# edwinyosorahardjo/compressjs-flattened

Hardware: AMD Instinct MI355X
Metric: bzip2 -9 compress MB/s at 1/2/4/8 MI355X; bit-exact output size vs ref (higher is better)
Workload: dtype u32; 1 GPU; Bzip2.compressFile level 9 (899981-byte blocks) on 1 x 100000000 bytes enwik8-shaped synthetic text (tools/textgen.c seed 1), device-resident; per_gpu_bytes=100000000, level=9, parallelism=1 GPU

## Files before the change

compressjs-flattened_amd/csrc/bwt.hip:

```cpp
#include "radix.hpp"
#include <stdlib.h>
#include <string.h>
#include <type_traits>

namespace cjs {

struct Geom { uint32_t nb, stride, n_last; };
__device__ __forceinline__ uint32_t blk_len(const Geom& g, uint32_t blk) { return blk == g.nb - 1 ? g.n_last : g.stride; }
struct VarGeom { uint32_t nb, stride, n_last; const uint32_t* len; };
__device__ __forceinline__ uint32_t blk_len(const VarGeom& g, uint32_t blk) { return g.len[blk]; }

template <typename G>
__global__ __launch_bounds__(256) void bwt_init_keys(const uint8_t* __restrict__ T, G g, int cyclic, int nsym, uint32_t M,
                                                     uint64_t* __restrict__ key, uint32_t* __restrict__ val) {
  for (uint64_t a = (uint64_t)blockIdx.x * 256 + threadIdx.x; a < M; a += (uint64_t)gridDim.x * 256) {
    const uint32_t blk = (uint32_t)(a / g.stride), i = (uint32_t)(a - (uint64_t)blk * g.stride), n = blk_len(g, blk);
    const uint8_t* t = T + (size_t)blk * g.stride;
    uint64_t k = 0;
    if constexpr (std::is_same_v<G, VarGeom>) {
      uint32_t x = i;
      if (i >= n) k = (1ull << (8 * nsym)) | i;
      else for (int j = 0; j < nsym; j++) { k = (k << 8) | t[x]; if (++x == n) x = 0; }
      k |= (uint64_t)blk << (8 * nsym + 1);
    } else if (cyclic) {
// ... 131 lines not shown
  const uint32_t single = nh & nx;
  uint32_t surv = (uint32_t)__popc(valid & ~single), heads = (uint32_t)__popc(nh & ~single);
  uint32_t last = nh ? (uint32_t)base + (uint32_t)tid * 16u + 32u - (uint32_t)__clz(nh) : 0u;
  {
    const uint64_t any = __ballot(nh != 0);
    const uint32_t run0 = (uint32_t)wave_id() * 2u;
    if (lane_id() == 0) {
      bool bad = false;
      for (uint32_t b = 0; b < 2; b++) bad |= base + (uint64_t)(run0 + b + 1u) * 512u <= A && (uint32_t)(any >> (32 * b)) == 0u;
      if (bad) atomicOr(big_flag, 1u);
    }
  }
  surv = block_sum<256>(surv, sm);
  heads = block_sum<256>(heads, sm);
  last = wave_max(last);
  if (lane_id() == 0) sm[wave_id()] = last;
  __syncthreads();
  if (tid == 0) {
    uint32_t m = sm[0]; for (int i = 1; i < 4; i++) m = sm[i] > m ? sm[i] : m;
    tile_cnt[blockIdx.x] = surv; tile_cnt[T + blockIdx.x] = heads; tile_cnt[2 * (size_t)T + blockIdx.x] = m;
  }
}

__global__ __launch_bounds__(1024) void bwt_scan_tiles(uint32_t* __restrict__ tile_cnt, uint32_t T, uint32_t* __restrict__ counters,
                                                      uint32_t* __restrict__ host_mirror ) {
  __shared__ uint32_t sm[16];
  __shared__ uint32_t mx[1024];
  uint32_t c0 = 0, c1 = 0, cm = 0;
  for (uint32_t base = 0; base < T; base += 1024) {
    const uint32_t i = base + threadIdx.x;
    const bool ok = i < T;
    uint32_t t0, t1;
    const uint32_t v0 = ok ? tile_cnt[i] : 0u, v1 = ok ? tile_cnt[T + i] : 0u, v2 = ok ? tile_cnt[2 * (size_t)T + i] : 0u;
    const uint32_t e0 = block_excl_sum<1024>(v0, sm, t0);
    const uint32_t e1 = block_excl_sum<1024>(v1, sm, t1);
    const uint32_t im = block_incl_max<1024>(v2, sm);
    mx[threadIdx.x] = im;
    __syncthreads();
    const uint32_t prev = threadIdx.x ? mx[threadIdx.x - 1] : 0u;
    const uint32_t chunk_max = mx[1023];
    __syncthreads();
    if (ok) {
      tile_cnt[i] = c0 + e0; tile_cnt[T + i] = c1 + e1;
      tile_cnt[2 * (size_t)T + i] = prev > cm ? prev : cm;
    }
    c0 += t0; c1 += t1; cm = chunk_max > cm ? chunk_max : cm;
  }
  if (threadIdx.x == 0) { counters[0] = c0; counters[1] = c1; host_mirror[0] = c0; host_mirror[1] = c1; host_mirror[4] = counters[4]; counters[4] = 0; }
}

__device__ __forceinline__ uint64_t class_head_before(const uint64_t* __restrict__ key, uint64_t seg0, uint64_t base, int shift, int lane) {
  if (base == seg0) return base;
  const uint64_t target = key[base] >> shift;
  const uint64_t off = base - seg0;
  const uint32_t back = off < 64u ? (uint32_t)off : 64u;
  const bool eq = (uint32_t)lane < back && (key[base - 1u - (uint32_t)lane] >> shift) == target;
  const uint64_t ne = ~__ballot(eq);
  const uint32_t m = ne ? (uint32_t)__builtin_ctzll(ne) : 64u;
  if (m < 64u || off <= 64u) return base - m;
  uint64_t lo = seg0, hi = base - 64u;
  while (hi > lo) {
    const uint64_t len = hi - lo, step = (len + 63u) / 64u, idx = lo + (uint64_t)lane * step;
    const bool hit = idx >= hi || (key[idx] >> shift) == target;
    const uint64_t hits = __ballot(hit);
    const uint32_t j = hits ? (uint32_t)__builtin_ctzll(hits) : 64u;
    if (!j) { hi = lo; break; }
    const uint64_t nhi = lo + (uint64_t)j * step;
    lo += (uint64_t)(j - 1u) * step + 1u;
    if (j < 64u && nhi < hi) hi = nhi;
  }
  return hi;
// ... 492 lines not shown
#pragma unroll
    for (int s = 0; s < 16; s++) {
      const uint32_t d = (comp[s] >> shift) & 255u;
      se[wcnt[w][d] + rk[s]] = ((uint64_t)comp[s] << 32) | pv[s];
    }
    __syncthreads();
#pragma unroll
    for (int s = 0; s < 16; s++) {
      const uint64_t e = se[(uint32_t)w * 1024u + (uint32_t)s * 64u + lane];
      comp[s] = (uint32_t)(e >> 32); pv[s] = (uint32_t)e;
    }
    __syncthreads();
  }
#pragma unroll
  for (int s = 0; s < 16; s++) {
    if ((ownm >> s) & 1u) {
      const uint32_t x = (uint32_t)w * 1024u + (uint32_t)s * 64u + lane;
      const uint32_t pc = x ? (uint32_t)(se[x - 1] >> 32) : ~comp[s];
      hflag[wb + x] = (uint8_t)((comp[s] != pc ? HF_NEW : 0u) | ((comp[s] >> 20) != (pc >> 20) ? HF_OLD : 0u));
      val[wb + x] = pv[s];
    }
  }
}
__global__ __launch_bounds__(1024) void scan_u32_single(uint32_t* __restrict__ arr, uint32_t n, uint32_t* __restrict__ total, uint32_t* __restrict__ host_total) {
  __shared__ uint32_t sm[16];
  uint32_t carry = 0;
  for (uint32_t base = 0; base < n; base += 1024) {
    const uint32_t i = base + threadIdx.x;
    uint32_t v = i < n ? arr[i] : 0u, tot;
    const uint32_t ex = block_excl_sum<1024>(v, sm, tot);
    if (i < n) arr[i] = carry + ex;
    carry += tot;
  }
  if (threadIdx.x == 0) { *total = carry; *host_total = carry; }
}
__device__ __forceinline__ void defer_flags(uint32_t A, const uint8_t* __restrict__ dflag, const uint64_t* __restrict__ key, uint64_t a0,
                                            uint32_t& f, uint32_t& heads, uint64_t (&k8)[8]) {
  f = 0; heads = 0;
  if (a0 >= A) return;
  if (a0 + 8 <= A) {
    const uint64_t w = *(const uint64_t*)(dflag + a0);
#pragma unroll
    for (int j = 0; j < 8; j++) f |= (uint32_t)((w >> (8 * j)) & 1ull) << j;
  } else for (int j = 0; j < 8; j++) if (a0 + j < A && dflag[a0 + j]) f |= 1u << j;
  if (!f) return;
#pragma unroll
  for (int j = 0; j < 8; j++) k8[j] = a0 + j < A ? key[a0 + j] : 0ull;
  const bool pf = a0 && dflag[a0 - 1];
  uint64_t prev = pf ? key[a0 - 1] >> 20 : ~0ull;
  bool prev_def = pf;
#pragma unroll
  for (int j = 0; j < 8; j++) {
    const bool d = (f >> j) & 1u;
    if (d && (!prev_def || prev != (k8[j] >> 20))) heads |= 1u << j;
    prev_def = d; prev = k8[j] >> 20;
  }
}
// ... 149 lines not shown
  if (tile >= Tn) return;
#pragma unroll 4
  for (int it = 0; it < 16; it++) {
    const uint64_t a = (uint64_t)tile * RS_TILE + (uint32_t)it * 256 + threadIdx.x;
    if (a >= M) break;
    const uint32_t blk = (uint32_t)(a / g.stride), p = (uint32_t)(a - (uint64_t)blk * g.stride), n = blk_len(g, blk);
    const uint8_t* t = T + (size_t)blk * g.stride;
    uint8_t* u = U + (size_t)blk * g.stride;
    const uint32_t s = __builtin_nontemporal_load(SA + a);
    const uint32_t p0 = R[(size_t)blk * g.stride];
    if (p == p0) u[0] = t[n - 1];
    else u[p < p0 ? p + 1 : p] = t[s - 1];
  }
}

enum Counter { CN_SURVIVORS = 0, CN_GROUPS = 1, CN_DEFERRED = 2, CN_DEFERRED_GROUPS = 3, CN_LARGE_GROUP = 4 };

size_t BwtWork::bytes_needed(size_t cap) {
  const size_t T = RadixWork::hist_tiles_for(cap);
  size_t b = 0;
  auto add = [&](size_t n) { b += (n + 255) & ~(size_t)255; };
  add(cap * 8); add(cap * 8); add(cap * 4); add(cap * 4); add(cap * 4); add(cap * 4); add(cap * 4);
  add(cap * 4); add(cap * 4); add(cap); add(cap);
  add(RadixWork::hist_words(T) * 4); add(256 * RadixWork::segs_for(cap) * 4); add(3 * T * 4); add(64);
  return b + 4096;
}
int BwtWork::carve(Arena& a, size_t cap_) {
  cap = cap_;
  const size_t T = RadixWork::hist_tiles_for(cap);
  key[0] = a.take<uint64_t>(cap); key[1] = a.take<uint64_t>(cap);
  val[0] = a.take<uint32_t>(cap); val[1] = a.take<uint32_t>(cap);
  pos[0] = a.take<uint32_t>(cap); pos[1] = a.take<uint32_t>(cap);
  gord = a.take<uint32_t>(cap);
  R = a.take<uint32_t>(cap); SA = a.take<uint32_t>(cap); dflag = a.take<uint8_t>(cap); hflag = a.take<uint8_t>(cap);
  CJS_TRY(rs.carve(a, T, RadixWork::segs_for(cap)));
  tile_cnt = a.take<uint32_t>(3 * T); counters = a.take<uint32_t>(16);
  if (!counters) return CJS_E_OUT_OF_MEMORY;
  if (!h_counters) CJS_HIP_TRY(hipHostMalloc((void**)h_counters.put(), 64));
  if (!ev_scan) CJS_HIP_TRY(hipEventCreateWithFlags(ev_scan.put(), hipEventDisableTiming));
  return 0;
}

struct Plan {
  bool segmented, packed;
  bool sweeps;
  int nsym, bits;
  int gs1, carried;
  SegGeom sg; GenSrc gen;
  const uint8_t* Tx; uint8_t* U;
};
template <typename G>
static Plan plan_round1(const BwtWork& w, const G& g, bool cyclic, const uint8_t* d_T, uint8_t* d_U) {
  constexpr bool VAR = std::is_same_v<G, VarGeom>;
  Plan p;
  const int sym_bits = cyclic ? 8 : 9;
  const uint32_t tps = ((g.nb > 1 ? g.stride : g.n_last) + RS_TILE - 1) / RS_TILE;
  p.segmented = !VAR && (uint64_t)g.nb * tps <= w.rs.hist_tiles && g.nb <= w.rs.bintot_segs && getenv("CJS_NO_SEGMENTED_SORT") == nullptr;
  p.packed = p.segmented && cyclic;
  p.sweeps = g.nb >= 8 && p.packed;
// ... 28 lines not shown
  hipLaunchKernelGGL(bwt_phase2_records, dim3(p.sg.nseg * p.sg.tps), dim3(256), 0, s, w.key[r.c], p.sg, p.gen.T, w.rs.hist, w.key[1 - r.c]);
  r.c = 1 - r.c;
  return radix_passes<uint64_t>(s, w.rs, w.key[0], w.val[0], w.key[1], w.val[1], r.c, r.A, 48, 64, lt, &p.sg, nullptr, true, true, w.dflag);
}

template <typename TG>
static void launch_tile_sort(hipStream_t s, uint32_t Tt, uint64_t* key, uint32_t* val, uint8_t* hflag, uint32_t A, uint8_t* dflag, uint32_t ngroups, const TG& tg) {
  if (ngroups && A / ngroups >= 5) hipLaunchKernelGGL(bwt_tile_sort_radix<TG>, dim3(xcd_grid(Tt)), dim3(256), 0, s, key, val, hflag, A, dflag, tg, Tt);
  else hipLaunchKernelGGL(bwt_tile_sort<TG>, dim3(xcd_grid(Tt)), dim3(256), 0, s, key, val, hflag, A, dflag, tg, Tt);
}
static int sort_round_whole(hipStream_t s, BwtWork& w, Round& r, LaunchTimes* lt) {
  CJS_TRY((radix_passes<uint64_t>(s, w.rs, w.key[0], w.val[0], w.key[1], w.val[1], r.c, r.A, 0, r.bits, lt)));
  hipLaunchKernelGGL(bwt_key_flags, dim3((r.A + 255) / 256 < 8192u ? (r.A + 255) / 256 : 8192u), dim3(256), 0, s, w.key[r.c], r.A, w.hflag);
  CJS_HIP_TRY(hipGetLastError());
  return 0;
}
static bool tile_sorted_round(uint32_t A) { return A >= 2 * TS_WIN; }
template <typename TG>
static int sort_round(hipStream_t s, BwtWork& w, Round& r, LaunchTimes* lt, const TG& tg) {
  if (!tile_sorted_round(r.A)) return sort_round_whole(s, w, r, lt);
  const uint32_t A = r.A, Tt = (A + TS_NOM - 1) / TS_NOM, Tg = (A + TS_GT - 1) / TS_GT;
  const int c = r.c;
  uint8_t* dflag = w.dflag;
  uint32_t* tcount = w.tile_cnt;
  if (r.no_large_groups) {
    launch_tile_sort(s, Tt, w.key[c], w.val[c], w.hflag, A, nullptr, r.ngroups, tg);
    CJS_HIP_TRY(hipGetLastError());
    return 0;
  }
  dev_fill(s, dflag, 1, A);
  launch_tile_sort(s, Tt, w.key[c], w.val[c], w.hflag, A, dflag, r.ngroups, tg);
  uint32_t* hcount = w.rs.hist;
  hipLaunchKernelGGL(bwt_defer_count, dim3(Tg), dim3(256), 0, s, A, dflag, w.key[c], tcount, hcount);
  hipLaunchKernelGGL(scan_u32_single, dim3(1), dim3(1024), 0, s, hcount, Tg, w.counters + CN_DEFERRED_GROUPS, w.h_counters + CN_DEFERRED_GROUPS);
  hipLaunchKernelGGL(scan_u32_single, dim3(1), dim3(1024), 0, s, tcount, Tg, w.counters + CN_DEFERRED, w.h_counters + CN_DEFERRED);
  CJS_HIP_TRY(hipStreamSynchronize(s));
  const uint32_t D = w.h_counters[CN_DEFERRED];
  if (env_debug()) fprintf(stderr, "[cjs bwt]   tile sort: %u of %u suffixes in groups > %u\n", D, A, TS_MAXGRP);
  if (D == 0) { r.no_large_groups = true; return 0; }
  if ((size_t)D > w.cap / 2) {
    const uint32_t Tk = (A + RS_TILE - 1) / RS_TILE;
    hipLaunchKernelGGL(bwt_gather_keys<decltype(tg.g)>, dim3(xcd_grid(Tk)), dim3(256), 0, s, tg.g, tg.cyclic, A, tg.h, tg.R, w.val[c], tg.pos, tg.gord, w.key[c], Tk);
    return sort_round_whole(s, w, r, lt);
  }
  uint64_t* dk0 = w.key[1 - c]; uint64_t* dk1 = dk0 + w.cap / 2;
  uint32_t* dv0 = w.val[1 - c]; uint32_t* dv1 = dv0 + w.cap / 2;
  uint32_t* dpos = w.pos[1 - r.pc];
  hipLaunchKernelGGL(bwt_defer_gather, dim3(Tg), dim3(256), 0, s, w.key[c], w.val[c], A, dflag, tcount, hcount, dk0, dv0, dpos);
  int cur = 0;
  const uint32_t ndg = w.h_counters[CN_DEFERRED_GROUPS];
  CJS_TRY((radix_passes<uint64_t>(s, w.rs, dk0, dv0, dk1, dv1, cur, D, 0, 20 + bits_for(ndg ? ndg - 1 : 0), lt)));
  hipLaunchKernelGGL(bwt_defer_scatter, dim3((D + 255) / 256 < 8192u ? (D + 255) / 256 : 8192u), dim3(256), 0, s, D, cur ? dk1 : dk0, cur ? dv1 : dv0, dpos,
                     w.hflag, w.val[c]);
  CJS_HIP_TRY(hipGetLastError());
  return 0;
}

template <bool FIRST, bool PACKED, int SWEEP, typename G>
static void launch_apply(hipStream_t s, BwtWork& w, const G& g, const Plan& p, const Round& r, uint32_t T) {
  hipLaunchKernelGGL((bwt_apply<FIRST, PACKED, SWEEP, G>), dim3(xcd_grid(T)), dim3(256), 0, s, FIRST ? w.key[r.c] : nullptr, FIRST ? nullptr : w.hflag,
                     w.val[r.c], w.pos[r.pc], r.A, g, w.tile_cnt, T, w.R, w.SA, w.val[1 - r.c], w.pos[1 - r.pc], w.gord, HalfMap{SWEEP ? 2u : 1u, g.stride},
                     p.Tx, p.U, w.counters + CN_LARGE_GROUP, p.gs1, p.carried);
}
template <typename G>
static int regroup(hipStream_t s, BwtWork& w, const G& g, const Plan& p, const Round& r) {
  const uint32_t T = (r.A + RS_TILE - 1) / RS_TILE;
  const bool first = r.rounds == 0, sweeps = first && p.sweeps;
  if (sweeps) launch_apply<true, true, 1>(s, w, g, p, r, T);
  else if (first) hipLaunchKernelGGL(bwt_flags, dim3(T), dim3(256), 0, s, w.key[r.c], r.A, w.tile_cnt, T, p.gs1, w.counters + CN_LARGE_GROUP, g.stride);
  else hipLaunchKernelGGL(bwt_flags_bytes, dim3(T), dim3(256), 0, s, w.hflag, r.A, w.tile_cnt, T, w.counters + CN_LARGE_GROUP);
  hipLaunchKernelGGL(bwt_scan_tiles, dim3(1), dim3(1024), 0, s, w.tile_cnt, T, w.counters, w.h_counters);
  CJS_HIP_TRY(hipEventRecord(w.ev_scan, s));
  if (sweeps) launch_apply<true, true, 2>(s, w, g, p, r, T);
  else if (first && p.packed) launch_apply<true, true, 0>(s, w, g, p, r, T);
  else if (first) launch_apply<true, false, 0>(s, w, g, p, r, T);
  else launch_apply<false, false, 0>(s, w, g, p, r, T);
  return 0;
}

template <typename G>
static void prepare_next(hipStream_t s, BwtWork& w, const G& g, bool cyclic, Round& r, TsGatherT<G>& tg) {
  if (tile_sorted_round(r.A)) tg = TsGatherT<G>{w.R, w.pos[r.pc], w.gord, r.h, (int)cyclic, g};
  else {
    const uint32_t Tg = (r.A + RS_TILE - 1) / RS_TILE;
    hipLaunchKernelGGL(bwt_gather_keys<G>, dim3(xcd_grid(Tg)), dim3(256), 0, s, g, (int)cyclic, r.A, r.h, w.R, w.val[r.c], w.pos[r.pc], w.gord, w.key[r.c], Tg);
  }
  r.h = r.h < (1u << 29) ? r.h * 2 : r.h;
  r.bits = 20 + bits_for(r.ngroups ? r.ngroups - 1 : 0);
}

template <typename G>
static int bwt_run_impl(hipStream_t s, BwtWork& w, const uint8_t* d_T, const G g, bool cyclic, uint8_t* d_U, uint32_t* d_pidx,
                        cjs_stats* stats, bool resolve_stats) {
  constexpr bool VAR = std::is_same_v<G, VarGeom>;
// ... 61 lines not shown
```

compressjs-flattened_amd/csrc/cjs_internal.h:

```cpp
#pragma once
#include <hip/hip_runtime.h>
#include <stdint.h>
#include <stddef.h>
#include <stdio.h>
#include <new>
#include "cjs_hip.h"

#define CJS_HIP_TRY(expr)                                                                   \
  do {                                                                                      \
    hipError_t _e = (expr);                                                                 \
    if (_e != hipSuccess) {                                                                 \
      fprintf(stderr, "[cjs_hip] %s failed: %s (%s:%d)\n", #expr, hipGetErrorString(_e), __FILE__, __LINE__); \
      return _e == hipErrorOutOfMemory ? CJS_E_OUT_OF_MEMORY : CJS_E_HIP;                    \
    }                                                                                       \
  } while (0)
#define CJS_TRY(expr) do { int _rc = (expr); if (_rc) return _rc; } while (0)

namespace cjs {

void clear_detail();
void set_detail(const char* fmt, ...);
bool env_debug(); bool env_no_ctx_cache();

#define CJS_GUARD_BEGIN try {
// ... 127 lines not shown
  }
};

struct SegGeom; struct GenSrc;
template <typename K>
int radix_passes(hipStream_t s, RadixWork& w, K* k0, uint32_t* v0, K* k1, uint32_t* v1, int& cur, uint32_t n, int lo_bit, int hi_bit,
                 LaunchTimes* lt = nullptr, const SegGeom* seg = nullptr, const GenSrc* gen = nullptr, bool noval = false,
                 bool first_hist_ready = false, uint8_t* dig = nullptr);
int radix_pass_segments(hipStream_t s, RadixWork& w, uint32_t* k0, uint32_t* v0, uint32_t* k1, uint32_t* v1, int& cur, uint32_t nseg, uint32_t stride,
                        int lo_bit, int hi_bit, bool noval, bool first_hist_ready);

struct BwtWork {
  size_t cap = 0;
  uint64_t* key[2] = {nullptr, nullptr};
  uint32_t* val[2] = {nullptr, nullptr};
  uint32_t* pos[2] = {nullptr, nullptr};
  uint32_t* gord = nullptr;
  uint32_t* R = nullptr;
  uint32_t* SA = nullptr;
  uint8_t* dflag = nullptr;
  uint8_t* hflag = nullptr;
  RadixWork rs;
  uint32_t* tile_cnt = nullptr;
  uint32_t* counters = nullptr;
  Pinned<uint32_t> h_counters;
  Event ev_scan;
  LaunchTimes lt;
  static size_t bytes_needed(size_t cap);
  int carve(Arena& a, size_t cap);
};

int bwt_run(hipStream_t s, BwtWork& w, const uint8_t* d_T, uint32_t nb, uint32_t stride, uint32_t n_last,
            bool cyclic, uint8_t* d_U, uint32_t* d_pidx, cjs_stats* stats, bool resolve_stats = true);
int bwt_run_var(hipStream_t s, BwtWork& w, const uint8_t* d_T, uint32_t nb, uint32_t stride, const uint32_t* d_len,
                uint8_t* d_U, uint32_t* d_pidx);
int ibwt_sentinel_run(hipStream_t s, const uint8_t* d_T, uint32_t max_len, uint32_t nb, const uint32_t* lens, const uint32_t* pidx, uint8_t* d_out);
struct MtfBufs;
int bwtc_model_launch(hipStream_t s, bool fast, const MtfBufs& mb, uint32_t nb, uint64_t* d_steps, size_t step_stride, uint32_t* d_nsteps);

}
```

compressjs-flattened_amd/csrc/huff.hip:

```cpp
#include "cjs_internal.h"
#include "prims.hpp"
#include "huff.h"

namespace cjs {

constexpr int MAXSYM = 258;
constexpr int MAX_BITS = 20;
constexpr int GSZ = 50;
constexpr int PD_GROUPS = 80;

__device__ uint64_t g_huff_clk[32];
__device__ uint64_t g_bt_clk[8];
#define BT_MARK(i) do { if (blockIdx.x == 0 && threadIdx.x == 0) g_bt_clk[i] = wall_clock64(); } while (0)
#define HB_MARK(i) do { if (dbg && blockIdx.x == 0 && threadIdx.x == 0) g_huff_clk[i] = wall_clock64(); } while (0)

__device__ __forceinline__ int ha_mod(int x, int len) { return x >= len ? x - len : x; }
__device__ __forceinline__ int ha_first(const int* a, int len, int i, int nodes_to_move) {
  const int limit = i;
  int k = len - 2;
  while (i >= nodes_to_move && ha_mod(a[i], len) > limit) { k = i; i -= (limit - i + 1); }
  if (i < nodes_to_move - 1) i = nodes_to_move - 1;
  while (k > i + 1) {
    const int mid = (i + k) >> 1;
    if (ha_mod(a[mid], len) > limit) k = mid; else i = mid;
// ... 252 lines not shown
          atomicAdd(&rep[(e1 / GSZ == gc ? sc : sd) * 260 + (ys[q] >> 16)], 1u);
        }
      }
    }
    if (i_hi >= npos) for (uint32_t i = nv * 8 + threadIdx.x; i < npos; i += 1024) atomicAdd(&rep[sel[i / GSZ] * 260 + A[i]], 1u);
  }
}

__device__ void block_accounting(HuffShared& S, HuffBufs& hb, uint32_t blk, const uint8_t* __restrict__ sel, uint8_t* __restrict__ selj,
                                 const uint16_t* __restrict__ bcost, const uint8_t* __restrict__ alist_all, uint32_t nsel, uint32_t asz, int n, int ng) {
  uint32_t data_bits = 0;
  {
    const uint32_t ntile = (nsel + PD_GROUPS - 1) / PD_GROUPS;
    uint32_t tsum = 0;
    if (threadIdx.x < ntile) {
      const uint32_t g1 = (threadIdx.x + 1) * PD_GROUPS < nsel ? (threadIdx.x + 1) * PD_GROUPS : nsel;
      for (uint32_t g = threadIdx.x * PD_GROUPS; g < g1; g++) tsum += bcost[g];
    }
    const uint32_t tex = block_excl_sum<1024>(tsum, S.sm, data_bits);
    if (threadIdx.x < ntile) hb.tileoff[(size_t)blk * hb.tile_stride + threadIdx.x] = tex;
  }
  uint32_t sel_bits = 0;
  {
    uint32_t lastc[6] = {0, 0, 0, 0, 0, 0};
    for (uint32_t base = 0; base < nsel; base += 1024) {
      const uint32_t g = base + threadIdx.x;
      const uint32_t sv = g < nsel ? sel[g] : 255u;
      uint32_t lastv[6];
#pragma unroll
      for (int v = 0; v < 6; v++) {
        const uint32_t mine = sv == (uint32_t)v ? g + 1 : 0u;
        const uint32_t im = block_incl_max<1024>(mine, S.sm);
        S.chist[threadIdx.x] = im;
        __syncthreads();
        const uint32_t ex = threadIdx.x ? S.chist[threadIdx.x - 1] : 0u;
        const uint32_t tmax = S.chist[1023];
        __syncthreads();
        lastv[v] = ex > lastc[v] ? ex : lastc[v];
        lastc[v] = tmax > lastc[v] ? tmax : lastc[v];
      }
      if (g < nsel) {
        uint32_t j = 0, mylast = 0;
#pragma unroll
        for (int v = 0; v < 6; v++) if ((uint32_t)v == sv) mylast = lastv[v];
#pragma unroll
        for (int v = 0; v < 6; v++) {
          if (v >= ng || (uint32_t)v == sv) continue;
          if (mylast) j += lastv[v] > mylast;
          else j += (lastv[v] != 0) || ((uint32_t)v < sv);
        }
        selj[g] = (uint8_t)j;
        sel_bits += j + 1;
      }
    }
  }
  sel_bits = block_sum<1024>(sel_bits, S.sm);
  uint32_t tab_bits = 0;
  for (int i = threadIdx.x; i < ng * n; i += 1024) {
    const int t = i / n, s = i - t * n;
    const int cur = S.lens[t][s], prev = s ? S.lens[t][s - 1] : cur;
    tab_bits += 2u * (uint32_t)(cur > prev ? cur - prev : prev - cur) + 1u + (s == 0 ? 5u : 0u);
  }
  tab_bits = block_sum<1024>(tab_bits, S.sm);
  if (threadIdx.x < 8) S.counts[threadIdx.x] = 0;
  __syncthreads();
  if (threadIdx.x < asz) atomicOr(&S.counts[0], 1u << (alist_all[(size_t)blk * 256 + threadIdx.x] >> 4));
  __syncthreads();
  const uint32_t nranges = (uint32_t)__builtin_popcount(S.counts[0]);
  uint8_t* glens = hb.lens + (size_t)blk * 6 * MAXSYM;
  uint32_t* gcodes = hb.codes + (size_t)blk * 6 * MAXSYM;
  for (int i = threadIdx.x; i < 6 * 32; i += 1024) (&S.key[0][0])[i] = 0;
  __syncthreads();
  uint32_t* lhist = &S.key[0][0];
  for (int i = threadIdx.x; i < ng * n; i += 1024) { const int t = i / n, s = i - t * n; atomicAdd(&lhist[t * 32 + S.lens[t][s]], 1u); }
  __syncthreads();
  if (threadIdx.x < (uint32_t)ng) {
// ... 445 lines not shown
```

compressjs-flattened_amd/csrc/prims.hpp:

```cpp
#pragma once
#include <hip/hip_runtime.h>
#include <stdint.h>

namespace cjs {

constexpr int WAVE = 64;

__device__ __forceinline__ int lane_id() { return threadIdx.x & 63; }
__device__ __forceinline__ int wave_id() { return threadIdx.x >> 6; }

template <int CTRL, int ROW_MASK>
__device__ __forceinline__ uint32_t dpp_move(uint32_t idv, uint32_t x) {
  return (uint32_t)__builtin_amdgcn_update_dpp((int)idv, (int)x, CTRL, ROW_MASK, 0xF, false);
}
constexpr int DPP_ROW_SHR1 = 0x111, DPP_ROW_SHR2 = 0x112, DPP_ROW_SHR4 = 0x114, DPP_ROW_SHR8 = 0x118, DPP_ROW_BCAST15 = 0x142, DPP_ROW_BCAST31 = 0x143;

template <typename Op>
__device__ __forceinline__ uint32_t wave_incl_scan_dpp(uint32_t x, uint32_t idv, Op op) {
  x = op(x, dpp_move<DPP_ROW_SHR1, 0xF>(idv, x));
  x = op(x, dpp_move<DPP_ROW_SHR2, 0xF>(idv, x));
  x = op(x, dpp_move<DPP_ROW_SHR4, 0xF>(idv, x));
  x = op(x, dpp_move<DPP_ROW_SHR8, 0xF>(idv, x));
  x = op(x, dpp_move<DPP_ROW_BCAST15, 0xA>(idv, x));
  x = op(x, dpp_move<DPP_ROW_BCAST31, 0xC>(idv, x));
// ... 81 lines not shown
    T s = lane < NW ? smem[lane] : T(0);
    s = wave_incl_max(s);
    if (lane < NW) smem[lane] = s;
  }
  __syncthreads();
  if (w) { T b = smem[w - 1]; incl = b > incl ? b : incl; }
  __syncthreads();
  return incl;
}
template <int BLOCK, typename T>
__device__ __forceinline__ T block_sum(T v, T* smem) {
  constexpr int NW = BLOCK / 64;
  const int lane = lane_id(), w = wave_id();
  T s = wave_sum(v);
  if (lane == 0) smem[w] = s;
  __syncthreads();
  T r = T(0);
#pragma unroll
  for (int i = 0; i < NW; i++) r += smem[i];
  __syncthreads();
  return r;
}

static __global__ __launch_bounds__(256) void dev_fill_kernel(uint4* __restrict__ p, uint32_t word, size_t n16) {
  const uint4 v = make_uint4(word, word, word, word);
  for (size_t i = (size_t)blockIdx.x * 256 + threadIdx.x; i < n16; i += (size_t)gridDim.x * 256) p[i] = v;
}
static inline void dev_fill(hipStream_t s, void* p, uint8_t byte, size_t bytes) {
  const size_t n16 = (bytes + 15) / 16;
  if (!n16) return;
  const size_t wg = (n16 + 255) / 256;
  hipLaunchKernelGGL(dev_fill_kernel, dim3((unsigned)(wg < 4096 ? wg : 4096)), dim3(256), 0, s, (uint4*)p, 0x01010101u * byte, n16);
}

}
```

compressjs-flattened_amd/csrc/radix.hip:

```cpp
#include "radix.hpp"

namespace cjs {

constexpr int HR = 8;
template <typename K, bool GEN>
__global__ __launch_bounds__(256) void rs_hist(const K* __restrict__ keys, SegGeom sg, GenSrc gs, int shift,
                                               uint32_t* __restrict__ hist, uint32_t T) {
  __shared__ uint32_t h[4 * 256 * HR];
  __shared__ __attribute__((aligned(16))) uint8_t tb[GEN ? RS_TILE + GEN_PAD + 16 : 16];
  const int tid = threadIdx.x;
  uint32_t* hw = h + (tid >> 6) * 256 * HR + (tid & (HR - 1));
#pragma unroll
  for (int i = 0; i < 4 * HR; i++) h[i * 256 + tid] = 0;
  const uint32_t tile = blockIdx.x;
  const TileRef t = tile_ref(sg, tile);
  uint32_t tb0 = 0;
  if (GEN) tb0 = gen_stage(gs, sg, t, tb);
  __syncthreads();
  if (GEN) {
#pragma unroll 4
    for (int it = 0; it < 16; it++) {
      const uint32_t loc = (uint32_t)it * 256 + tid;
      if (loc < t.nvalid) atomicAdd(&hw[((uint32_t)(gen_key(gs, sg, t, tb, tb0, loc) >> shift) & 255u) * HR], 1u);
    }
// ... 38 lines not shown
  uint32_t wv[5];
#pragma unroll
  for (int j = 0; j < 5; j++) {
    const uint32_t wi = (uint32_t)j * 256u + tid;
    wv[j] = (t.nvalid && (uintptr_t)(al + wi) < a1) ? al[wi] : 0u;
  }
  __syncthreads();
#pragma unroll
  for (int j = 0; j < 5; j++) {
    const uintptr_t wa = (uintptr_t)(al + ((uint32_t)j * 256u + tid));
#pragma unroll
    for (int b = 0; b < 4; b++)
      if (wa + b >= a0 && wa + b < a1) atomicAdd(&hw[((wv[j] >> (8 * b)) & 255u) * HB], 1u);
  }
  __syncthreads();
  uint32_t sum = 0;
#pragma unroll
  for (int i = 0; i < 4; i++)
#pragma unroll
    for (int r = 0; r < HB; r++) sum += h[i * 256 * HB + tid * HB + r];
  hist[(size_t)tile * 256 + tid] = sum;
}

__global__ __launch_bounds__(256) void rs_scan_bins(uint32_t* __restrict__ hist, uint32_t tps, uint32_t* __restrict__ bintot) {
  uint32_t* p = hist + (size_t)blockIdx.x * tps * 256 + threadIdx.x;
  uint32_t carry = 0;
  uint32_t i = 0;
  for (; i + 8 <= tps; i += 8) {
    uint32_t v[8];
#pragma unroll
    for (int j = 0; j < 8; j++) v[j] = p[(size_t)(i + j) * 256];
#pragma unroll
    for (int j = 0; j < 8; j++) { p[(size_t)(i + j) * 256] = carry; carry += v[j]; }
  }
  for (; i < tps; i++) { const uint32_t v = p[(size_t)i * 256]; p[(size_t)i * 256] = carry; carry += v; }
  bintot[(size_t)blockIdx.x * 256 + threadIdx.x] = carry;
}
constexpr uint32_t SB_CHUNK = 64;
__global__ __launch_bounds__(256) void rs_scan_chunk_sum(const uint32_t* __restrict__ hist, uint32_t T, uint32_t* __restrict__ csum) {
  const uint32_t t0 = blockIdx.x * SB_CHUNK, t1 = t0 + SB_CHUNK < T ? t0 + SB_CHUNK : T;
  uint32_t acc = 0;
  for (uint32_t t = t0; t < t1; t++) acc += hist[(size_t)t * 256 + threadIdx.x];
  csum[(size_t)blockIdx.x * 256 + threadIdx.x] = acc;
}
__global__ __launch_bounds__(256) void rs_scan_chunk_mid(uint32_t* __restrict__ csum, uint32_t nch, uint32_t* __restrict__ bintot) {
  uint32_t carry = 0;
  for (uint32_t c = 0; c < nch; c++) { const uint32_t v = csum[(size_t)c * 256 + threadIdx.x]; csum[(size_t)c * 256 + threadIdx.x] = carry; carry += v; }
  bintot[threadIdx.x] = carry;
}
__global__ __launch_bounds__(256) void rs_scan_chunk_apply(uint32_t* __restrict__ hist, uint32_t T, const uint32_t* __restrict__ csum) {
  const uint32_t t0 = blockIdx.x * SB_CHUNK, t1 = t0 + SB_CHUNK < T ? t0 + SB_CHUNK : T;
  uint32_t carry = csum[(size_t)blockIdx.x * 256 + threadIdx.x];
  for (uint32_t t = t0; t < t1; t++) { const uint32_t v = hist[(size_t)t * 256 + threadIdx.x]; hist[(size_t)t * 256 + threadIdx.x] = carry; carry += v; }
}

template <typename K, bool GEN, bool NOVAL>
__global__ __launch_bounds__(256) void rs_scatter(const K* __restrict__ kin, const uint32_t* __restrict__ vin,
                                                  K* __restrict__ kout, uint32_t* __restrict__ vout, SegGeom sg, GenSrc gs, int shift,
                                                  const uint32_t* __restrict__ hist, uint32_t T, const uint32_t* __restrict__ bintot,
                                                  uint8_t* __restrict__ dig ) {
  __shared__ __attribute__((aligned(16))) K skey[RS_TILE + 2];
// ... 63 lines not shown
      if (dig) dig[dst] = (uint8_t)((uint64_t)kk >> (shift + 8));
    }
  }
}

template <typename K>
int radix_passes(hipStream_t s, RadixWork& w, K* k0, uint32_t* v0, K* k1, uint32_t* v1, int& cur, uint32_t n, int lo_bit, int hi_bit,
                 LaunchTimes* lt, const SegGeom* seg, const GenSrc* gen, bool noval, bool first_hist_ready, uint8_t* dig) {
  const uint32_t T1 = (n + RS_TILE - 1) / RS_TILE;
  const SegGeom sg = seg ? *seg : SegGeom{1u, n, n, T1};
  const uint32_t T = sg.nseg * sg.tps;
  if (T > w.hist_tiles || sg.nseg > w.bintot_segs) return CJS_E_INVALID_ARG;
  K* kk[2] = {k0, k1}; uint32_t* vv[2] = {v0, v1};
  const GenSrc g0{nullptr, 0, 0, 0};
  for (int shift = lo_bit; shift < hi_bit; shift += 8) {
    const bool first_gen = gen && shift == lo_bit;
    const bool dig_out = dig && shift + 8 < hi_bit;
    if (first_hist_ready && shift == lo_bit) {}
    else if (dig && shift != lo_bit) hipLaunchKernelGGL(rs_hist_bytes, dim3(T), dim3(256), 0, s, dig, sg, w.hist, 0u);
    else if (first_gen && gen->cyclic && gen->packed && shift == PK_KEY_LO)
      hipLaunchKernelGGL(rs_hist_bytes, dim3(T), dim3(256), 0, s, gen->T, sg, w.hist, 6u);
    else if (first_gen) hipLaunchKernelGGL((rs_hist<K, true>), dim3(T), dim3(256), 0, s, kk[cur], sg, *gen, shift, w.hist, T);
    else hipLaunchKernelGGL((rs_hist<K, false>), dim3(T), dim3(256), 0, s, kk[cur], sg, g0, shift, w.hist, T);
    if (sg.tps <= 4 * SB_CHUNK) hipLaunchKernelGGL(rs_scan_bins, dim3(sg.nseg), dim3(256), 0, s, w.hist, sg.tps, w.bintot);
    else {
      for (uint32_t sgi = 0; sgi < sg.nseg; sgi++) {
        uint32_t* hseg = w.hist + (size_t)sgi * sg.tps * 256;
        const uint32_t nch = (sg.tps + SB_CHUNK - 1) / SB_CHUNK;
        uint32_t* csum = w.hist + (size_t)w.hist_tiles * 256;
        hipLaunchKernelGGL(rs_scan_chunk_sum, dim3(nch), dim3(256), 0, s, hseg, sg.tps, csum);
        hipLaunchKernelGGL(rs_scan_chunk_mid, dim3(1), dim3(256), 0, s, csum, nch, w.bintot + (size_t)sgi * 256);
        hipLaunchKernelGGL(rs_scan_chunk_apply, dim3(nch), dim3(256), 0, s, hseg, sg.tps, csum);
      }
    }
    if (lt) lt->begin(s, n);
#define RS_SCATTER(GEN_, NOVAL_, G_) hipLaunchKernelGGL((rs_scatter<K, GEN_, NOVAL_>), dim3(T), dim3(256), 0, s, kk[cur], vv[cur], kk[1 - cur], vv[1 - cur], sg, G_, shift, w.hist, T, w.bintot, dig_out ? dig : nullptr)
    if (noval) { if (first_gen) RS_SCATTER(true, true, *gen); else RS_SCATTER(false, true, g0); }
    else { if (first_gen) RS_SCATTER(true, false, *gen); else RS_SCATTER(false, false, g0); }
#undef RS_SCATTER
    if (lt) lt->end(s);
    cur = 1 - cur;
  }
  CJS_HIP_TRY(hipGetLastError());
  return 0;
}
template int radix_passes<uint64_t>(hipStream_t, RadixWork&, uint64_t*, uint32_t*, uint64_t*, uint32_t*, int&, uint32_t, int, int, LaunchTimes*,
                                    const SegGeom*, const GenSrc*, bool, bool, uint8_t*);
// ... 17 lines not shown
```

Measured before the change: 9174 MB/s.

## Parallelize single-block tile scans across blocks and split serial scan loops

Replaces the single-block looping tile-count scan and deferred-count scans with multi-block kernels: each block re-reduces all preceding elements to get its carry, then scans its own chunk into a separate output buffer. The two deferred scans are merged into one launch via a 2D grid, rs_scan_bins splits each bin's serial scan across four thread quarters with a two-pass reduce/apply, and the Huffman selector MTF scan is changed from one block-wide max-scan per 1024 selectors to per-thread contiguous ranges with a single cross-thread scan. The aim is to remove long serial latency chains in small bookkeeping kernels. In exchange, the redundant prefix re-reading grows quadratically with tile count, and tile_cnt doubles in size to hold the separate scan output.

```diff
diff --git a/compressjs-flattened_amd/csrc/bwt.hip b/compressjs-flattened_amd/csrc/bwt.hip
--- a/compressjs-flattened_amd/csrc/bwt.hip
+++ b/compressjs-flattened_amd/csrc/bwt.hip
@@ -177,31 +177,39 @@
   }
 }
 
-__global__ __launch_bounds__(1024) void bwt_scan_tiles(uint32_t* __restrict__ tile_cnt, uint32_t T, uint32_t* __restrict__ counters,
+__global__ __launch_bounds__(1024) void bwt_scan_tiles(const uint32_t* __restrict__ tile_cnt, uint32_t* __restrict__ scan, uint32_t T,
+                                                      uint32_t* __restrict__ counters,
                                                       uint32_t* __restrict__ host_mirror ) {
   __shared__ uint32_t sm[16];
   __shared__ uint32_t mx[1024];
+  const uint32_t base = blockIdx.x * 1024u;
   uint32_t c0 = 0, c1 = 0, cm = 0;
-  for (uint32_t base = 0; base < T; base += 1024) {
-    const uint32_t i = base + threadIdx.x;
-    const bool ok = i < T;
-    uint32_t t0, t1;
-    const uint32_t v0 = ok ? tile_cnt[i] : 0u, v1 = ok ? tile_cnt[T + i] : 0u, v2 = ok ? tile_cnt[2 * (size_t)T + i] : 0u;
-    const uint32_t e0 = block_excl_sum<1024>(v0, sm, t0);
-    const uint32_t e1 = block_excl_sum<1024>(v1, sm, t1);
-    const uint32_t im = block_incl_max<1024>(v2, sm);
-    mx[threadIdx.x] = im;
-    __syncthreads();
-    const uint32_t prev = threadIdx.x ? mx[threadIdx.x - 1] : 0u;
-    const uint32_t chunk_max = mx[1023];
-    __syncthreads();
-    if (ok) {
-      tile_cnt[i] = c0 + e0; tile_cnt[T + i] = c1 + e1;
-      tile_cnt[2 * (size_t)T + i] = prev > cm ? prev : cm;
-    }
-    c0 += t0; c1 += t1; cm = chunk_max > cm ? chunk_max : cm;
-  }
-  if (threadIdx.x == 0) { counters[0] = c0; counters[1] = c1; host_mirror[0] = c0; host_mirror[1] = c1; host_mirror[4] = counters[4]; counters[4] = 0; }
+  if (base) {
+#pragma unroll 4
+    for (uint32_t i = threadIdx.x; i < base; i += 1024) {
+      const uint32_t v2 = tile_cnt[2 * (size_t)T + i];
+      c0 += tile_cnt[i]; c1 += tile_cnt[T + i]; cm = v2 > cm ? v2 : cm;
+    }
+    c0 = block_sum<1024>(c0, sm); c1 = block_sum<1024>(c1, sm); cm = block_max<1024>(cm, sm);
+  }
+  const uint32_t i = base + threadIdx.x;
+  const bool ok = i < T;
+  uint32_t t0, t1;
+  const uint32_t v0 = ok ? tile_cnt[i] : 0u, v1 = ok ? tile_cnt[T + i] : 0u, v2 = ok ? tile_cnt[2 * (size_t)T + i] : 0u;
+  const uint32_t e0 = block_excl_sum<1024>(v0, sm, t0);
+  const uint32_t e1 = block_excl_sum<1024>(v1, sm, t1);
+  const uint32_t im = block_incl_max<1024>(v2, sm);
+  mx[threadIdx.x] = im;
+  __syncthreads();
+  const uint32_t prev = threadIdx.x ? mx[threadIdx.x - 1] : 0u;
+  if (ok) {
+    scan[i] = c0 + e0; scan[T + i] = c1 + e1;
+    scan[2 * (size_t)T + i] = prev > cm ? prev : cm;
+  }
+  if (blockIdx.x == gridDim.x - 1 && threadIdx.x == 0) {
+    c0 += t0; c1 += t1;
+    counters[0] = c0; counters[1] = c1; host_mirror[0] = c0; host_mirror[1] = c1; host_mirror[4] = counters[4]; counters[4] = 0;
+  }
 }
 
 __device__ __forceinline__ uint64_t class_head_before(const uint64_t* __restrict__ key, uint64_t seg0, uint64_t base, int shift, int lane) {
@@ -740,17 +748,24 @@
     }
   }
 }
-__global__ __launch_bounds__(1024) void scan_u32_single(uint32_t* __restrict__ arr, uint32_t n, uint32_t* __restrict__ total, uint32_t* __restrict__ host_total) {
+struct ScanPair { const uint32_t* in[2]; uint32_t* out[2]; uint32_t* total[2]; uint32_t* host_total[2]; };
+__global__ __launch_bounds__(1024) void scan_u32_pair(ScanPair sp, uint32_t n) {
   __shared__ uint32_t sm[16];
+  const bool y = blockIdx.y != 0;
+  const uint32_t* __restrict__ in = y ? sp.in[1] : sp.in[0];
+  uint32_t* __restrict__ out = y ? sp.out[1] : sp.out[0];
+  const uint32_t base = blockIdx.x * 1024u;
   uint32_t carry = 0;
-  for (uint32_t base = 0; base < n; base += 1024) {
-    const uint32_t i = base + threadIdx.x;
-    uint32_t v = i < n ? arr[i] : 0u, tot;
-    const uint32_t ex = block_excl_sum<1024>(v, sm, tot);
-    if (i < n) arr[i] = carry + ex;
-    carry += tot;
-  }
-  if (threadIdx.x == 0) { *total = carry; *host_total = carry; }
+  if (base) {
+#pragma unroll 4
+    for (uint32_t i = threadIdx.x; i < base; i += 1024) carry += in[i];
+    carry = block_sum<1024>(carry, sm);
+  }
+  const uint32_t i = base + threadIdx.x;
+  uint32_t v = i < n ? in[i] : 0u, tot;
+  const uint32_t ex = block_excl_sum<1024>(v, sm, tot);
+  if (i < n) out[i] = carry + ex;
+  if (blockIdx.x == gridDim.x - 1 && threadIdx.x == 0) { *(y ? sp.total[1] : sp.total[0]) = carry + tot; *(y ? sp.host_total[1] : sp.host_total[0]) = carry + tot; }
 }
 __device__ __forceinline__ void defer_flags(uint32_t A, const uint8_t* __restrict__ dflag, const uint64_t* __restrict__ key, uint64_t a0,
                                             uint32_t& f, uint32_t& heads, uint64_t (&k8)[8]) {
@@ -946,7 +961,7 @@
   auto add = [&](size_t n) { b += (n + 255) & ~(size_t)255; };
   add(cap * 8); add(cap * 8); add(cap * 4); add(cap * 4); add(cap * 4); add(cap * 4); add(cap * 4);
   add(cap * 4); add(cap * 4); add(cap); add(cap);
-  add(RadixWork::hist_words(T) * 4); add(256 * RadixWork::segs_for(cap) * 4); add(3 * T * 4); add(64);
+  add(RadixWork::hist_words(T) * 4); add(256 * RadixWork::segs_for(cap) * 4); add(6 * T * 4); add(64);
   return b + 4096;
 }
 int BwtWork::carve(Arena& a, size_t cap_) {
@@ -958,7 +973,7 @@
   gord = a.take<uint32_t>(cap);
   R = a.take<uint32_t>(cap); SA = a.take<uint32_t>(cap); dflag = a.take<uint8_t>(cap); hflag = a.take<uint8_t>(cap);
   CJS_TRY(rs.carve(a, T, RadixWork::segs_for(cap)));
-  tile_cnt = a.take<uint32_t>(3 * T); counters = a.take<uint32_t>(16);
+  tile_cnt = a.take<uint32_t>(6 * T); tile_scan = tile_cnt ? tile_cnt + 3 * T : nullptr; counters = a.take<uint32_t>(16);
   if (!counters) return CJS_E_OUT_OF_MEMORY;
   if (!h_counters) CJS_HIP_TRY(hipHostMalloc((void**)h_counters.put(), 64));
   if (!ev_scan) CJS_HIP_TRY(hipEventCreateWithFlags(ev_scan.put(), hipEventDisableTiming));
@@ -1033,7 +1048,7 @@
   const uint32_t A = r.A, Tt = (A + TS_NOM - 1) / TS_NOM, Tg = (A + TS_GT - 1) / TS_GT;
   const int c = r.c;
   uint8_t* dflag = w.dflag;
-  uint32_t* tcount = w.tile_cnt;
+  uint32_t* tcount = w.tile_scan;
   if (r.no_large_groups) {
     launch_tile_sort(s, Tt, w.key[c], w.val[c], w.hflag, A, nullptr, r.ngroups, tg);
     CJS_HIP_TRY(hipGetLastError());
@@ -1041,10 +1056,11 @@
   }
   dev_fill(s, dflag, 1, A);
   launch_tile_sort(s, Tt, w.key[c], w.val[c], w.hflag, A, dflag, r.ngroups, tg);
-  uint32_t* hcount = w.rs.hist;
-  hipLaunchKernelGGL(bwt_defer_count, dim3(Tg), dim3(256), 0, s, A, dflag, w.key[c], tcount, hcount);
-  hipLaunchKernelGGL(scan_u32_single, dim3(1), dim3(1024), 0, s, hcount, Tg, w.counters + CN_DEFERRED_GROUPS, w.h_counters + CN_DEFERRED_GROUPS);
-  hipLaunchKernelGGL(scan_u32_single, dim3(1), dim3(1024), 0, s, tcount, Tg, w.counters + CN_DEFERRED, w.h_counters + CN_DEFERRED);
+  uint32_t* hraw = w.rs.hist; uint32_t* hcount = hraw + Tg;
+  hipLaunchKernelGGL(bwt_defer_count, dim3(Tg), dim3(256), 0, s, A, dflag, w.key[c], w.tile_cnt, hraw);
+  hipLaunchKernelGGL(scan_u32_pair, dim3((Tg + 1023) / 1024, 2), dim3(1024), 0, s,
+                     ScanPair{{hraw, w.tile_cnt}, {hcount, tcount}, {w.counters + CN_DEFERRED_GROUPS, w.counters + CN_DEFERRED},
+                              {w.h_counters + CN_DEFERRED_GROUPS, w.h_counters + CN_DEFERRED}}, Tg);
   CJS_HIP_TRY(hipStreamSynchronize(s));
   const uint32_t D = w.h_counters[CN_DEFERRED];
   if (env_debug()) fprintf(stderr, "[cjs bwt]   tile sort: %u of %u suffixes in groups > %u\n", D, A, TS_MAXGRP);
@@ -1070,7 +1086,7 @@
 template <bool FIRST, bool PACKED, int SWEEP, typename G>
 static void launch_apply(hipStream_t s, BwtWork& w, const G& g, const Plan& p, const Round& r, uint32_t T) {
   hipLaunchKernelGGL((bwt_apply<FIRST, PACKED, SWEEP, G>), dim3(xcd_grid(T)), dim3(256), 0, s, FIRST ? w.key[r.c] : nullptr, FIRST ? nullptr : w.hflag,
-                     w.val[r.c], w.pos[r.pc], r.A, g, w.tile_cnt, T, w.R, w.SA, w.val[1 - r.c], w.pos[1 - r.pc], w.gord, HalfMap{SWEEP ? 2u : 1u, g.stride},
+                     w.val[r.c], w.pos[r.pc], r.A, g, SWEEP == 1 ? w.tile_cnt : w.tile_scan, T, w.R, w.SA, w.val[1 - r.c], w.pos[1 - r.pc], w.gord, HalfMap{SWEEP ? 2u : 1u, g.stride},
                      p.Tx, p.U, w.counters + CN_LARGE_GROUP, p.gs1, p.carried);
 }
 template <typename G>
@@ -1080,7 +1096,7 @@
   if (sweeps) launch_apply<true, true, 1>(s, w, g, p, r, T);
   else if (first) hipLaunchKernelGGL(bwt_flags, dim3(T), dim3(256), 0, s, w.key[r.c], r.A, w.tile_cnt, T, p.gs1, w.counters + CN_LARGE_GROUP, g.stride);
   else hipLaunchKernelGGL(bwt_flags_bytes, dim3(T), dim3(256), 0, s, w.hflag, r.A, w.tile_cnt, T, w.counters + CN_LARGE_GROUP);
-  hipLaunchKernelGGL(bwt_scan_tiles, dim3(1), dim3(1024), 0, s, w.tile_cnt, T, w.counters, w.h_counters);
+  hipLaunchKernelGGL(bwt_scan_tiles, dim3((T + 1023) / 1024), dim3(1024), 0, s, w.tile_cnt, w.tile_scan, T, w.counters, w.h_counters);
   CJS_HIP_TRY(hipEventRecord(w.ev_scan, s));
   if (sweeps) launch_apply<true, true, 2>(s, w, g, p, r, T);
   else if (first && p.packed) launch_apply<true, true, 0>(s, w, g, p, r, T);
diff --git a/compressjs-flattened_amd/csrc/cjs_internal.h b/compressjs-flattened_amd/csrc/cjs_internal.h
--- a/compressjs-flattened_amd/csrc/cjs_internal.h
+++ b/compressjs-flattened_amd/csrc/cjs_internal.h
@@ -173,6 +173,7 @@
   uint8_t* hflag = nullptr;
   RadixWork rs;
   uint32_t* tile_cnt = nullptr;
+  uint32_t* tile_scan = nullptr;
   uint32_t* counters = nullptr;
   Pinned<uint32_t> h_counters;
   Event ev_scan;
diff --git a/compressjs-flattened_amd/csrc/huff.hip b/compressjs-flattened_amd/csrc/huff.hip
--- a/compressjs-flattened_amd/csrc/huff.hip
+++ b/compressjs-flattened_amd/csrc/huff.hip
@@ -298,36 +298,37 @@
   }
   uint32_t sel_bits = 0;
   {
-    uint32_t lastc[6] = {0, 0, 0, 0, 0, 0};
-    for (uint32_t base = 0; base < nsel; base += 1024) {
-      const uint32_t g = base + threadIdx.x;
-      const uint32_t sv = g < nsel ? sel[g] : 255u;
-      uint32_t lastv[6];
+    const uint32_t per = (nsel + 1023) / 1024;
+    const uint32_t g0 = threadIdx.x * per < nsel ? threadIdx.x * per : nsel, g1 = g0 + per < nsel ? g0 + per : nsel;
+    uint32_t lastv[6] = {0, 0, 0, 0, 0, 0};
+    for (uint32_t g = g0; g < g1; g++) {
+      const uint32_t sv = sel[g];
+#pragma unroll
+      for (int v = 0; v < 6; v++) if (sv == (uint32_t)v) lastv[v] = g + 1;
+    }
+#pragma unroll
+    for (int v = 0; v < 6; v++) {
+      const uint32_t im = block_incl_max<1024>(lastv[v], S.sm);
+      S.chist[threadIdx.x] = im;
+      __syncthreads();
+      lastv[v] = threadIdx.x ? S.chist[threadIdx.x - 1] : 0u;
+      __syncthreads();
+    }
+    for (uint32_t g = g0; g < g1; g++) {
+      const uint32_t sv = sel[g];
+      uint32_t j = 0, mylast = 0;
+#pragma unroll
+      for (int v = 0; v < 6; v++) if ((uint32_t)v == sv) mylast = lastv[v];
 #pragma unroll
       for (int v = 0; v < 6; v++) {
-        const uint32_t mine = sv == (uint32_t)v ? g + 1 : 0u;
-        const uint32_t im = block_incl_max<1024>(mine, S.sm);
-        S.chist[threadIdx.x] = im;
-        __syncthreads();
-        const uint32_t ex = threadIdx.x ? S.chist[threadIdx.x - 1] : 0u;
-        const uint32_t tmax = S.chist[1023];
-        __syncthreads();
-        lastv[v] = ex > lastc[v] ? ex : lastc[v];
-        lastc[v] = tmax > lastc[v] ? tmax : lastc[v];
+        if (v >= ng || (uint32_t)v == sv) continue;
+        if (mylast) j += lastv[v] > mylast;
+        else j += (lastv[v] != 0) || ((uint32_t)v < sv);
       }
-      if (g < nsel) {
-        uint32_t j = 0, mylast = 0;
-#pragma unroll
-        for (int v = 0; v < 6; v++) if ((uint32_t)v == sv) mylast = lastv[v];
-#pragma unroll
-        for (int v = 0; v < 6; v++) {
-          if (v >= ng || (uint32_t)v == sv) continue;
-          if (mylast) j += lastv[v] > mylast;
-          else j += (lastv[v] != 0) || ((uint32_t)v < sv);
-        }
-        selj[g] = (uint8_t)j;
-        sel_bits += j + 1;
-      }
+      selj[g] = (uint8_t)j;
+      sel_bits += j + 1;
+#pragma unroll
+      for (int v = 0; v < 6; v++) if ((uint32_t)v == sv) lastv[v] = g + 1;
     }
   }
   sel_bits = block_sum<1024>(sel_bits, S.sm);
diff --git a/compressjs-flattened_amd/csrc/prims.hpp b/compressjs-flattened_amd/csrc/prims.hpp
--- a/compressjs-flattened_amd/csrc/prims.hpp
+++ b/compressjs-flattened_amd/csrc/prims.hpp
@@ -127,6 +127,20 @@
   return r;
 }
 
+template <int BLOCK, typename T>
+__device__ __forceinline__ T block_max(T v, T* smem) {
+  constexpr int NW = BLOCK / 64;
+  const int lane = lane_id(), w = wave_id();
+  T s = wave_max(v);
+  if (lane == 0) smem[w] = s;
+  __syncthreads();
+  T r = smem[0];
+#pragma unroll
+  for (int i = 1; i < NW; i++) r = smem[i] > r ? smem[i] : r;
+  __syncthreads();
+  return r;
+}
+
 static __global__ __launch_bounds__(256) void dev_fill_kernel(uint4* __restrict__ p, uint32_t word, size_t n16) {
   const uint4 v = make_uint4(word, word, word, word);
   for (size_t i = (size_t)blockIdx.x * 256 + threadIdx.x; i < n16; i += (size_t)gridDim.x * 256) p[i] = v;
diff --git a/compressjs-flattened_amd/csrc/radix.hip b/compressjs-flattened_amd/csrc/radix.hip
--- a/compressjs-flattened_amd/csrc/radix.hip
+++ b/compressjs-flattened_amd/csrc/radix.hip
@@ -84,21 +84,41 @@
   hist[(size_t)tile * 256 + tid] = sum;
 }
 
-__global__ __launch_bounds__(256) void rs_scan_bins(uint32_t* __restrict__ hist, uint32_t tps, uint32_t* __restrict__ bintot) {
-  uint32_t* p = hist + (size_t)blockIdx.x * tps * 256 + threadIdx.x;
+constexpr int SBB = 16;
+__global__ __launch_bounds__(1024) void rs_scan_bins(uint32_t* __restrict__ hist, uint32_t tps, uint32_t* __restrict__ bintot) {
+  __shared__ uint32_t part[4][256];
+  const uint32_t d = threadIdx.x & 255u, q = threadIdx.x >> 8;
+  const uint32_t per = (tps + 3) / 4;
+  const uint32_t r0 = q * per < tps ? q * per : tps, r1 = r0 + per < tps ? r0 + per : tps;
+  uint32_t* p = hist + (size_t)blockIdx.x * tps * 256 + d;
+  uint32_t sum = 0;
+  for (uint32_t i = r0; i < r1; i += SBB) {
+    uint32_t v[SBB];
+#pragma unroll
+    for (int j = 0; j < SBB; j++) v[j] = i + j < r1 ? p[(size_t)(i + j) * 256] : 0u;
+#pragma unroll
+    for (int j = 0; j < SBB; j++) sum += v[j];
+  }
+  part[q][d] = sum;
+  __syncthreads();
   uint32_t carry = 0;
-  uint32_t i = 0;
-  for (; i + 8 <= tps; i += 8) {
-    uint32_t v[8];
-#pragma unroll
-    for (int j = 0; j < 8; j++) v[j] = p[(size_t)(i + j) * 256];
-#pragma unroll
-    for (int j = 0; j < 8; j++) { p[(size_t)(i + j) * 256] = carry; carry += v[j]; }
-  }
-  for (; i < tps; i++) { const uint32_t v = p[(size_t)i * 256]; p[(size_t)i * 256] = carry; carry += v; }
-  bintot[(size_t)blockIdx.x * 256 + threadIdx.x] = carry;
+#pragma unroll
+  for (uint32_t j = 0; j < 3; j++) if (j < q) carry += part[j][d];
+  for (uint32_t i = r0; i < r1; i += SBB) {
+    uint32_t v[SBB];
+#pragma unroll
+    for (int j = 0; j < SBB; j++) v[j] = i + j < r1 ? p[(size_t)(i + j) * 256] : 0u;
+#pragma unroll
+    for (int j = 0; j < SBB; j++) { if (i + j < r1) p[(size_t)(i + j) * 256] = carry; carry += v[j]; }
+  }
+  if (q == 3) bintot[(size_t)blockIdx.x * 256 + d] = carry;
 }
 constexpr uint32_t SB_CHUNK = 64;
+constexpr uint32_t SB_ONE_LAUNCH = 576;
+static uint32_t scan_one_launch_tiles() {
+  static const uint32_t lim = [] { const char* e = getenv("CJS_SCAN_ONE_LAUNCH_TILES"); return e ? (uint32_t)strtoul(e, nullptr, 10) : SB_ONE_LAUNCH; }();
+  return lim;
+}
 __global__ __launch_bounds__(256) void rs_scan_chunk_sum(const uint32_t* __restrict__ hist, uint32_t T, uint32_t* __restrict__ csum) {
   const uint32_t t0 = blockIdx.x * SB_CHUNK, t1 = t0 + SB_CHUNK < T ? t0 + SB_CHUNK : T;
   uint32_t acc = 0;
@@ -208,7 +228,7 @@
       hipLaunchKernelGGL(rs_hist_bytes, dim3(T), dim3(256), 0, s, gen->T, sg, w.hist, 6u);
     else if (first_gen) hipLaunchKernelGGL((rs_hist<K, true>), dim3(T), dim3(256), 0, s, kk[cur], sg, *gen, shift, w.hist, T);
     else hipLaunchKernelGGL((rs_hist<K, false>), dim3(T), dim3(256), 0, s, kk[cur], sg, g0, shift, w.hist, T);
-    if (sg.tps <= 4 * SB_CHUNK) hipLaunchKernelGGL(rs_scan_bins, dim3(sg.nseg), dim3(256), 0, s, w.hist, sg.tps, w.bintot);
+    if (sg.tps <= scan_one_launch_tiles()) hipLaunchKernelGGL(rs_scan_bins, dim3(sg.nseg), dim3(1024), 0, s, w.hist, sg.tps, w.bintot);
     else {
       for (uint32_t sgi = 0; sgi < sg.nseg; sgi++) {
         uint32_t* hseg = w.hist + (size_t)sgi * sg.tps * 256;
```

Measured after the change: 9336 MB/s (median of 6 runs). 1.02x the previous value.
